# rafaelvp-db/databricks-distributed-deep-learning

Measured on AMD Instinct MI355X. Metric: ResNet-50 images/sec (whole node), higher is better.
Workload: dtype bf16

## Files before the change

### csrc/include/ddl_lds.h

```cpp
#pragma once
#include "ddl_common.h"

typedef __attribute__((address_space(3))) void lds_void;
typedef __attribute__((address_space(3))) s16x4 lds_v4;
typedef uint32_t u32x2 __attribute__((ext_vector_type(2)));
typedef uint32_t u32x4 __attribute__((ext_vector_type(4)));

#define BARRIER() __builtin_amdgcn_s_barrier()
#define LGKM0() asm volatile("s_waitcnt lgkmcnt(0)" ::: "memory")
#define VMN(n) asm volatile("s_waitcnt vmcnt(" #n ")" ::: "memory")

__device__ __forceinline__ void wait_vm(int n) {
    switch (n) {
        case 0: asm volatile("s_waitcnt vmcnt(0)" ::: "memory"); break;
        case 1: asm volatile("s_waitcnt vmcnt(1)" ::: "memory"); break;
        case 2: asm volatile("s_waitcnt vmcnt(2)" ::: "memory"); break;
        case 6: asm volatile("s_waitcnt vmcnt(6)" ::: "memory"); break;
        case 7: asm volatile("s_waitcnt vmcnt(7)" ::: "memory"); break;
        case 8: asm volatile("s_waitcnt vmcnt(8)" ::: "memory"); break;
        default: asm volatile("s_waitcnt vmcnt(0)" ::: "memory"); break;
    }
}

__device__ __forceinline__ bf16x8 ds_read16(uint32_t addr) {
    bf16x8 v;
    asm volatile("ds_read_b128 %0, %1" : "=v"(v) : "v"(addr));
    return v;
}
template <int OFF>
__device__ __forceinline__ bf16x8 ds_read16_off(uint32_t addr) {
    bf16x8 v;
    asm volatile("ds_read_b128 %0, %1 offset:%2" : "=v"(v) : "v"(addr), "i"(OFF));
    return v;
}
__device__ __forceinline__ uint2 ds_read8(uint32_t addr) {
    uint2 v;
    asm volatile("ds_read_b64 %0, %1" : "=v"(v) : "v"(addr));
    return v;
}
__device__ __forceinline__ uint32_t ds_read32(uint32_t addr) {
    uint32_t v;
    asm volatile("ds_read_b32 %0, %1" : "=v"(v) : "v"(addr));
    return v;
}
__device__ __forceinline__ void ds_write8(uint32_t addr, uint2 v) {
    asm volatile("ds_write_b64 %0, %1" ::"v"(addr), "v"(v) : "memory");
}
__device__ __forceinline__ void ds_write16(uint32_t addr, u32x4 v) {
    asm volatile("ds_write_b128 %0, %1" ::"v"(addr), "v"(v) : "memory");
}
__device__ __forceinline__ s16x4 ds_read_tr8(uint32_t addr) {
    s16x4 v;
    asm volatile("ds_read_b64_tr_b16 %0, %1" : "=v"(v) : "v"(addr));
    return v;
}
__device__ __forceinline__ bf16x8 tr_frag(uint32_t a, uint32_t b) {
    const s16x4 lo = ds_read_tr8(a), hi = ds_read_tr8(b);
    typedef short s16x8 __attribute__((ext_vector_type(8)));
    const s16x8 r = {lo[0], lo[1], lo[2], lo[3], hi[0], hi[1], hi[2], hi[3]};
    return __builtin_bit_cast(bf16x8, r);
}

__device__ __forceinline__ s16x4 lds_read_tr(lds_v4* __restrict__ p) {
    return __builtin_amdgcn_ds_read_tr16_b64_v4i16(p);
}

__device__ __forceinline__ void glds16(const void* g, char* dst) {
    __builtin_amdgcn_global_load_lds(g, (lds_void*)dst, 16, 0, 0);
}
__device__ __forceinline__ void glds16_nt(const void* g, char* dst) {
    __builtin_amdgcn_global_load_lds(g, (lds_void*)dst, 16, 0, 2);
}
__device__ __forceinline__ void glds4(const void* g, char* dst) {
    __builtin_amdgcn_global_load_lds(g, (lds_void*)dst, 4, 0, 0);
}
__device__ __forceinline__ __amdgpu_buffer_rsrc_t rsrc(const void* p, uint32_t bytes) {
    return __builtin_amdgcn_make_buffer_rsrc(const_cast<void*>(p), 0, (int)bytes, 0x00020000);
}

__device__ __forceinline__ int swz_kc(int b) { return b ^ (((b >> 9) & 1) << 5); }
__device__ __forceinline__ int swz_ko(int r) { return 2 * ((r & 3) | (((r >> 3) & 1) << 2)); }
__device__ __forceinline__ bf16x8 frag_ko(const char* img, int col_base, int lane) {
    const int g = lane >> 4, q = (lane >> 2) & 3, pq = lane & 3;
    const int chunk = (col_base + 4 * pq) >> 3;
    const int ra = 8 * g + q, rb = ra + 4;
    const s16x4 lo = lds_read_tr((lds_v4*)(img + ra * 256 + ((chunk ^ swz_ko(ra)) << 4) + (pq & 1) * 8));
    const s16x4 hi = lds_read_tr((lds_v4*)(img + rb * 256 + ((chunk ^ swz_ko(rb)) << 4) + (pq & 1) * 8));
    typedef short s16x8 __attribute__((ext_vector_type(8)));
    const s16x8 r = {lo[0], lo[1], lo[2], lo[3], hi[0], hi[1], hi[2], hi[3]};
    return __builtin_bit_cast(bf16x8, r);
}

template <int W>
constexpr int swm() { return W / 8 >= 16 ? 15 : W / 8 - 1; }

template <int NWAVES, int W, int NROWS, long LD = W>
__device__ __forceinline__ void dma_rows(const bf16_t* src, long row0, long rows_valid, char* dst, int wv, int lane) {
    constexpr int CPR = W / 8;
    constexpr int RPI = CPR >= 64 ? 1 : 64 / CPR;
    constexpr int IPR = CPR >= 64 ? CPR / 64 : 1;
    constexpr int NINST = NROWS * IPR / RPI;
    static_assert(NINST % NWAVES == 0, "instructions split evenly over the waves");
#pragma unroll
    for (int qq = 0; qq < NINST / NWAVES; ++qq) {
        const int q = qq * NWAVES + wv;
        const int r = (q / IPR) * RPI + (CPR >= 64 ? 0 : lane / CPR);
        const int cl = CPR >= 64 ? (q % IPR) * 64 + lane : lane % CPR;
        const int c = cl ^ (r & swm<W>());
        const long gr = min(row0 + r, rows_valid - 1);
        glds16_nt(src + gr * LD + c * 8, dst + q * 1024);
    }
}
```

### csrc/kernels/conv3_bwd.hip

```cpp
#include "ddl_lds.h"

#include <algorithm>

namespace {

constexpr int NW = 8, NTH = NW * 64;
constexpr int TM = 32;
constexpr int DPT = 6, SPT = 1;

struct C3Params {
    const bf16_t* dz;
    const bf16_t* x3;
    const float* mean3;
    const float* istd3;
    const float* coef3;
    const bf16_t* a2;
    const bf16_t* x2;
    const uint8_t* mask2;
    const float* mean2;
    const float* istd2;
    const bf16_t* wt;
    bf16_t* dz2;
    float* colstats;
    bf16_t* wpart;
    long M;
    int tiles, chunk;
    uint32_t dz2_bytes;
};

__device__ __forceinline__ u32x4 bn_apply8(bf16x8 dzv, bf16x8 xv, const float* A, const float* B, const float* D,
                                           bool valid) {
    const u32x4 gw = __builtin_bit_cast(u32x4, dzv), xw = __builtin_bit_cast(u32x4, xv);
    const uint32_t keep = valid ? ~0u : 0u;
    u32x4 o;
#pragma unroll
    for (int i = 0; i < 4; ++i) {
        const float g0 = lo_f(gw[i]), g1 = hi_f(gw[i]);
        const float x0 = lo_f(xw[i]), x1 = hi_f(xw[i]);
        const float o0 = bn_bwd_apply1(A[2 * i], g0, B[2 * i], x0, D[2 * i]);
        const float o1 = bn_bwd_apply1(A[2 * i + 1], g1, B[2 * i + 1], x1, D[2 * i + 1]);
        o[i] = pack2bf(o0, o1) & keep;
    }
    return o;
}

template <int CO, int CI, int NBUF>
__global__ __launch_bounds__(NTH, 1) void conv3_bwd_k(C3Params p) {
    static_assert(CO == 256 && CI == 64 && (NBUF == 2 || NBUF == 3), "shape");
    constexpr int WBYTES = CI * CO * 2, ZBYTES = TM * CO * 2, ABYTES = TM * CI * 2;
    constexpr int O_DZ = 0, O_X3 = ZBYTES, O_A2 = 2 * ZBYTES, O_X2 = O_A2 + ABYTES, O_MK = O_X2 + ABYTES;
    constexpr int BUFB = O_MK + 1024;
    constexpr int LDS = WBYTES + NBUF * BUFB;
    static_assert(LDS <= 160 * 1024, "LDS");
    __shared__ __attribute__((aligned(16))) char smem[LDS];
    const int tid = threadIdx.x, lane = tid & 63, wv = __builtin_amdgcn_readfirstlane(tid >> 6);
    const int g = lane >> 4, r16 = lane & 15;
    const uint32_t lds0 = (uint32_t)(uintptr_t)smem;
    const __amdgpu_buffer_rsrc_t crs = rsrc(p.dz2, p.dz2_bytes);
    const int t0 = blockIdx.x * p.chunk, t1 = min(p.tiles, t0 + p.chunk);

    auto prefetch = [&](int t, int buf) {
        char* base = smem + WBYTES + buf * BUFB;
        const long m0 = (long)t * TM;
#pragma unroll
        for (int qq = 0; qq < 2; ++qq) {
            const int q = qq * NW + wv, r = q * 2 + (lane >> 5), c = (lane & 31) ^ (r & 15);
            const long gr = min(m0 + r, p.M - 1);
            glds16_nt(p.dz + gr * CO + c * 8, base + O_DZ + q * 1024);
            glds16_nt(p.x3 + gr * CO + c * 8, base + O_X3 + q * 1024);
        }
        {
            const int q = wv & 3, r = q * 8 + (lane >> 3), c = (lane & 7) ^ (r & 7);
            const long gr = min(m0 + r, p.M - 1);
            glds16_nt((wv < 4 ? p.a2 : p.x2) + gr * CI + c * 8, base + (wv < 4 ? O_A2 : O_X2) + q * 1024);
        }
        {
            const long b = min(m0 * (CI / 8) + lane * 4, p.M * (CI / 8) - 4);
            const uint8_t* src = p.mask2 ? p.mask2 + b : (const uint8_t*)p.a2;
            glds4(src, base + O_MK);
        }
    };
#pragma unroll
    for (int qq = 0; qq < CI / 2 / NW; ++qq) {
        const int q = qq * NW + wv, r = q * 2 + (lane >> 5), c = (lane & 31) ^ (r & 15);
        glds16_nt(p.wt + (long)r * CO + c * 8, smem + q * 1024);
    }
#pragma unroll
    for (int u = 0; u < NBUF - 1; ++u)
        if (t0 + u < t1) prefetch(t0 + u, u);

    const int tc = tid & 31, tr = tid >> 5;
    float cA[8], cB[8], cD[8];
    bn_bwd_apply_coefs8(p.mean3, p.istd3, p.coef3, CO, tc * 8, cA, cB, cD);
    const uint32_t toff = tr * (CO * 2) + ((tc ^ tr) << 4);

    const int dj = wv & 3;
    const bool dgw = wv < 4;
    uint32_t aoff[2][CO / 32], boff[CO / 32];
#pragma unroll
    for (int kk = 0; kk < CO / 32; ++kk) {
        const int rb = 16 * dj + r16;
        boff[kk] = lds0 + rb * (CO * 2) + (((kk * 4 + g) ^ (rb & 15)) << 4);
#pragma unroll
        for (int i = 0; i < 2; ++i) {
            const int ra = 16 * i + r16;
            aoff[i][kk] = ra * (CO * 2) + (((kk * 4 + g) ^ (ra & 15)) << 4);
        }
    }
    uint32_t coff[2], moff[2];
// ... 86 lines not shown
            }
        }
        LGKM0();
        __builtin_amdgcn_sched_barrier(0);
        {
            typedef short s16x8 __attribute__((ext_vector_type(8)));
            bf16x8 fa[2], fb[4];
#pragma unroll
            for (int i = 0; i < 2; ++i) {
                const s16x8 r = {fal[i][0][0], fal[i][0][1], fal[i][0][2], fal[i][0][3],
                                 fal[i][1][0], fal[i][1][1], fal[i][1][2], fal[i][1][3]};
                fa[i] = __builtin_bit_cast(bf16x8, r);
            }
#pragma unroll
            for (int j = 0; j < 4; ++j) {
                const s16x8 r = {fbl[j][0][0], fbl[j][0][1], fbl[j][0][2], fbl[j][0][3],
                                 fbl[j][1][0], fbl[j][1][1], fbl[j][1][2], fbl[j][1][3]};
                fb[j] = __builtin_bit_cast(bf16x8, r);
            }
#pragma unroll
            for (int i = 0; i < 2; ++i)
#pragma unroll
                for (int j = 0; j < 4; ++j)
                    wacc[i][j] = __builtin_amdgcn_mfma_f32_16x16x32_bf16(fb[j], fa[i], wacc[i][j], 0, 0, 0);
        }
        if (dgw) {
#pragma unroll
            for (int i = 0; i < 2; ++i) {
                float v[4] = {acc[i][0], acc[i][1], acc[i][2], acc[i][3]};
                const float xv[4] = {lo_f(ev[i].x), hi_f(ev[i].x), lo_f(ev[i].y), hi_f(ev[i].y)};
                const uint32_t bits = mword[i] >> mshift;
#pragma unroll
                for (int e = 0; e < 4; ++e) v[e] = ((bits >> e) & 1u) ? v[e] : 0.f;
                const uint32_t lo = pack2bf(v[0], v[1]), hi = pack2bf(v[2], v[3]);
                ds_write8(img + O_X2 + coff[i], make_uint2(lo, hi));
                if (m0 + 16 * i + r16 < p.M) {
                    const float tq[4] = {lo_f(lo), hi_f(lo), lo_f(hi), hi_f(hi)};
#pragma unroll
                    for (int e = 0; e < 4; ++e) {
                        st_s[e] += tq[e];
                        st_q[e] = __builtin_fmaf(tq[e], xv[e], st_q[e]);
                    }
                }
            }
        }
        LGKM0();
        __builtin_amdgcn_s_barrier();
        {
            const int row = 4 * wv + (lane >> 4), pc = lane & 15;
            const uint2 d = ds_read8(img + O_X2 + row * (CI * 2) + (((pc >> 1) ^ (row & 7)) << 4) + (pc & 1) * 8);
            LGKM0();
            __builtin_amdgcn_sched_barrier(0);
            const long grow = m0 + row;
            const uint32_t off = grow < p.M ? (uint32_t)((grow * CI + pc * 4) * 2) : 0x80000000u;
            __builtin_amdgcn_raw_buffer_store_b64(__builtin_bit_cast(u32x2, d), crs, (int)off, 0, 0);
        }
        buf = buf + 1 == NBUF ? 0 : buf + 1;
    }
    asm volatile("s_waitcnt vmcnt(0)" ::: "memory");
    __syncthreads();

    bf16_t* wout = p.wpart + (long)blockIdx.x * CO * CI;
#pragma unroll
    for (int i = 0; i < 2; ++i)
#pragma unroll
        for (int j = 0; j < 4; ++j)
            *reinterpret_cast<uint2*>(wout + (long)(32 * wv + 16 * i + r16) * CI + 16 * j + 4 * g) =
                make_uint2(pack2bf(wacc[i][j][0], wacc[i][j][1]), pack2bf(wacc[i][j][2], wacc[i][j][3]));

    if (dgw) {
#pragma unroll
        for (int e = 0; e < 4; ++e) {
            const float a = row16_sum(st_s[e]), b = row16_sum(st_q[e]);
            if (r16 == 0) {
                const int col = 16 * dj + 4 * g + e;
                p.colstats[(long)blockIdx.x * 2 * CI + col] = a;
                p.colstats[(long)blockIdx.x * 2 * CI + CI + col] =
                    __builtin_fmaf(-p.mean2[col], a, b) * p.istd2[col];
            }
        }
    }
}

}

DDL_API int ddl_conv3_bwd_grid(long M, int grid) {
    const int tiles64 = (int)((M + 63) / 64);
    const int g = std::min(grid > 0 ? std::min(grid, 256) : 256, tiles64);
    const int chunk64 = (tiles64 + g - 1) / g;
    return (tiles64 + chunk64 - 1) / chunk64;
}

DDL_API int ddl_conv3_bwd(const void* dz, const void* x3, const float* mean3, const float* istd3, const float* coef3,
                          const void* a2, const void* x2, const uint8_t* mask2, const float* mean2, const float* istd2,
                          const void* wt, void* dz2, float* colstats, void* wpart, long wpart_elems, void* dW,
                          int dw_f32, int accumulate, long M, int Cout, int Cin, int grid, hipStream_t st) {
    if (Cout != 256 || Cin != 64 || M < 1 || M * (long)Cout * 2 >= (1l << 31)) return -1;
    if (!dz || !x3 || !mean3 || !istd3 || !coef3 || !a2 || !x2 || !mean2 || !istd2 || !wt || !dz2 || !colstats ||
        !wpart || !dW)
        return -1;
    for (const void* q : {dz, x3, a2, x2, wt, (const void*)dz2, (const void*)wpart})
        if ((uintptr_t)q & 15) return -1;
    if ((uintptr_t)dW & (dw_f32 ? 15 : 7)) return -1;
    C3Params p{};
    p.dz = (const bf16_t*)dz;
    p.x3 = (const bf16_t*)x3;
    p.mean3 = mean3;
    p.istd3 = istd3;
    p.coef3 = coef3;
    p.a2 = (const bf16_t*)a2;
    p.x2 = (const bf16_t*)x2;
    p.mask2 = mask2;
    p.mean2 = mean2;
    p.istd2 = istd2;
    p.wt = (const bf16_t*)wt;
    p.dz2 = (bf16_t*)dz2;
    p.colstats = colstats;
    p.wpart = (bf16_t*)wpart;
    p.M = M;
    p.tiles = (int)((M + TM - 1) / TM);
    const int G = ddl_conv3_bwd_grid(M, grid);
    p.chunk = 2 * (((int)((M + 63) / 64) + G - 1) / G);
    p.dz2_bytes = (uint32_t)(M * Cin * 2);
    if (wpart_elems < (long)G * Cout * Cin) return -1;
    hipLaunchKernelGGL((conv3_bwd_k<256, 64, 3>), dim3(G), dim3(NTH), 0, st, p);
    ddl_wgrad_reduce(p.wpart, G, Cout, Cin, dW, Cin, accumulate, dw_f32, st);
    const hipError_t e = hipGetLastError();
    if (e != hipSuccess) return -2 - (int)e;
    return G;
}
```

### databricks_distributed_deep_learning_amd/ops/_lib.py

```python
from __future__ import annotations

import ctypes
import os
from typing import Optional

import torch

_PKG_DIR = os.path.dirname(os.path.dirname(os.path.abspath(__file__)))
LIB_PATH = os.environ.get("DDL_NATIVE_LIB") or os.path.join(_PKG_DIR, "_native", "libddl_kernels.so")

_lib: Optional[ctypes.CDLL] = None
_load_error: Optional[str] = None
_mode = os.environ.get("DDL_NATIVE", "auto").lower()


class NativeUnavailable(RuntimeError):
    pass


def set_mode(mode: str) -> None:
    global _mode
    if mode not in ("auto", "on", "off"):
        raise ValueError(mode)
    _mode = mode
# ... 38 lines not shown
def load_error() -> Optional[str]:
    load()
    return _load_error


def use_native(*tensors: torch.Tensor) -> bool:
    if _mode == "off":
        return False
    if not all(t is None or t.is_cuda for t in tensors):
        return False
    if load() is None:
        raise NativeUnavailable(
            f"HIP kernel library unavailable on a GPU run: {_load_error}. "
            "Build it with `python csrc/build.py` or set DDL_NATIVE=off for stock PyTorch ops.")
    return True


def get() -> ctypes.CDLL:
    lib = load()
    if lib is None:
        raise NativeUnavailable(_load_error)
    return lib


def stream() -> ctypes.c_void_p:
    return ctypes.c_void_p(torch.cuda.current_stream().cuda_stream)


def ptr(t: Optional[torch.Tensor]) -> ctypes.c_void_p:
    return ctypes.c_void_p(0 if t is None else t.data_ptr())


def check(rc: int, what: str) -> None:
    if rc != 0:
        raise RuntimeError(f"native kernel {what} failed with HIP error {rc}")


P, I, L, F, U64 = ctypes.c_void_p, ctypes.c_int, ctypes.c_long, ctypes.c_float, ctypes.c_uint64
_SIGS = {
    "ddl_bn_stats_nblk": [L, I],
    "ddl_bn_bwd_nblk": [L, I],
    "ddl_bn_rows_sum": [P, I, I, P, P, P],
    "ddl_rows_sum_sink": [I, P, I, I, I, P, I, P, P],
    "ddl_bn_stats_partials": [I, P, L, I, P, P],
    "ddl_bn_bwd_partials": [I, P, P, P, P, P, L, I, I, P, P],
    "ddl_bn_bwd_finish": [I, P, P, P, P, P, P, L, L, I, I, P, P, P, P, P, P, P, I, P],
    "ddl_bn_bwd_from_partials": [I, P, I, P, L, P, P, P, P, P, L, I, P, P, P, P, P, I, P],
    "ddl_bn_partials_ws": [I, I],
    "ddl_bn_fwd_train": [I, P, L, I, P, P, P, P, F, F, P, P, P, P, P, P],
    "ddl_bn_eval_coeffs": [I, I, P, P, P, P, F, P, P, P],
    "ddl_bn_apply": [I, P, P, P, P, P, L, I, I, P, P],
    "ddl_bn_apply2": [I, P, P, P, P, P, P, P, L, I, I, P, P],
    "ddl_bn_relu_maxpool": [I, P, P, P, P, P, P, I, I, I, I, I, I, P],
    "ddl_bn_bwd_pool_nblk": [],
    "ddl_bn_bwd_pool": [I, P, P, P, P, P, P, P, I, I, I, I, I, I, P, P, P, P, P, I, P],
    "ddl_bn_bwd_coef_from_partials": [I, P, I, P, L, P, P, L, I, P, P, P, I, P],
    "ddl_bn_bwd_apply_coef": [I, P, P, P, P, P, L, I, P, P],
    "ddl_bn_fwd_from_partials": [I, P, I, L, I, P, P, P, P, F, F, P, P, P, P, P, L],
    "ddl_conv_w_dgrad": [P, P, I, I, I, I, I, I, P, P, P],
    "ddl_conv_w_dgrad_batch": [P, P, I, P],
    "ddl_gelu_bwd_colsum": [I, P, P, P, L, I, P, P, I, I, P],
    "ddl_acc_f32": [I, P, P, L, P],
    "ddl_tanh_bwd": [I, P, P, P, L, P],
    "ddl_copy2d": [I, P, L, L, L, P, L, L, L, P],
    "ddl_add_into": [I, P, P, L, P],
    "ddl_zero": [P, L, P],
    "ddl_rows_add_row": [I, P, P, P, L, L, P],
    "ddl_seq_prepend_add": [I, P, P, P, P, L, L, L, P],
    "ddl_sort_ids_ok": [L, L],
    "ddl_sort_ids": [P, L, P, P, P],
    "ddl_drain_acc": [I, P, P, L, P],
    "ddl_acc_grad": [I, P, P, L, I, I, P],
    "ddl_softmax_topk": [I, P, L, I, I, P, P, P, P],
    "ddl_gemm_conv_multi": [I, I, P, P, P, P, P, L, I, P, P],
    "ddl_conv3x3": [P, P, P, I, I, I, I, I, P, P, P, P, P, P, I, P],
    "ddl_conv3x3_wgrad": [P, P, P, I, I, I, I, I, P, L, I, I, I, P],
    "ddl_stem_wgrad": [P, P, P, I, I, I, I, I, I, I, P, L, I, I, I, P],
    "ddl_stem_fwd": [P, P, P, I, I, I, I, P, I, P],
    "ddl_s2d_input": [P, I, I, I, I, I, P, I, I, P],
    "ddl_s2d_weight": [P, I, I, I, I, P, I, I, P],
    "ddl_skinny_gemm": [P, P, P, L, I, I, P, P, P, P, P, P, I, P],
    "ddl_stream_gemm": [P, P, P, L, I, I, P, P, P, P, P, P, I, P],
    "ddl_stream_wgrad_ws": [I, I],
    "ddl_conv3_bwd_grid": [L, I],
    "ddl_conv3_bwd": [P, P, P, P, P, P, P, P, P, P, P, P, P, P, L, P, I, I, L, I, I, I, P],
    "ddl_bn_bwd": [I, P, P, P, P, P, P, L, I, I, P, P, P, P, P, P, I, P],
    "ddl_ln_supported": [I],
    "ddl_ln_fwd": [I, P, P, L, P, P, P, P, P, L, I, F, U64, F, P],
    "ddl_ln_bwd_nblk": [L],
    "ddl_ln_bwd": [I, P, P, P, L, P, P, P, P, P, P, P, L, I, I, P, U64, F, P, P, P, P],
    "ddl_gelu_fwd": [I, P, P, L, P],
    "ddl_gelu_bwd": [I, P, P, P, L, P],
    "ddl_dropout": [I, P, P, L, U64, F, P],
    "ddl_colsum_nblk": [L],
    "ddl_colsum": [I, P, L, I, P, P, I, I, P],
    "ddl_softmax_ce": [I, P, P, L, I, P, P, P, P],
    "ddl_scale_by": [I, P, P, P, L, P],
    "ddl_maxpool_fwd": [I, P, P, P, I, I, I, I, I, I, I, I, I, P],
    "ddl_maxpool_bwd": [I, P, P, P, I, I, I, I, I, I, I, I, I, P],
    "ddl_avgpool_fwd": [I, P, P, I, I, I, P],
    "ddl_avgpool_bwd": [I, P, P, I, I, I, P],
    "ddl_embedding_fwd": [I, P, P, P, L, I, P],
    "ddl_embedding_bwd": [I, P, P, P, P, L, L, I, I, P],
    "ddl_embedding_bwd_sorted": [I, P, P, P, P, P, L, I, I, P],
    "ddl_sgd_step": [I, P, P, I, P, P, P, I, P, F, F, F, I, I, P],
    "ddl_adamw_step": [I, P, P, I, P, P, P, P, I, P, F, F, F, F, F, F, F, F, F, P],
    "ddl_lamb_step": [I, P, P, I, P, P, P, P, I, P, F, F, F, F, F, F, F, F, F, P, P],
    "ddl_sumsq": [I, P, L, P, P],
    "ddl_lamb_phase1": [I, P, P, P, P, P, I, P, F, F, F, F, F, F, F, F, P, P],
    "ddl_lamb_phase2": [P, I, P, P, P, P, I, F, F, F, F, F, P, P],
}
_fns = {}


def fn(name: str):
    f = _fns.get(name)
    if f is None:
        f = getattr(get(), name)
        if name in _SIGS:
            f.argtypes = _SIGS[name]
        f.restype = ctypes.c_int
        _fns[name] = f
    return f


def call(name: str, *args) -> None:
    rc = fn(name)(*args, stream())
    if rc != 0:
        raise RuntimeError(f"native kernel {name} failed with code {rc}")


def register(sigs: dict) -> None:
    _SIGS.update(sigs)


def dcode(t: torch.Tensor) -> int:
    if t.dtype == torch.bfloat16:
        return 1
    if t.dtype == torch.float32:
        return 0
    raise TypeError(f"native kernels support fp32/bf16, got {t.dtype}")


def p(t: Optional[torch.Tensor]) -> int:
    return 0 if t is None else t.data_ptr()


def grad_sink(param) -> Optional[torch.Tensor]:
    if param is None:
        return None
    return getattr(param, "_ddl_main_grad", None)


def grad_ready(param) -> None:
    cb = getattr(param, "_ddl_grad_ready", None)
    if cb is not None:
        cb()


import contextlib as _contextlib

_WGRAD_STREAM = os.environ.get("DDL_WGRAD_STREAM", "0") != "0"
_side: dict = {}


def wgrad_stream_enabled() -> bool:
    return _WGRAD_STREAM
# ... 36 lines not shown
```

### databricks_distributed_deep_learning_amd/ops/_native_conv.py

```python
from __future__ import annotations

import ctypes
import os

import torch
import torch.nn.functional as F

from . import _lib
from ._lib import grad_ready, grad_sink
from ._native_gemm import MODE_CONV, MODE_CONVW, MODE_NN, MODE_NT, MODE_TN, gemm, plan, stats_rows_max
from ._native_norm import _BN_BWD_EPI, _BN_BWD_EPI_RES


def _desc(N, H, W, C, P, Q, stride, h_off, w_off, h_step, w_step, R, S, OH, OW, ostep=1, oa=0, ob=0):
    return [N, H, W, C, P, Q, stride, h_off, w_off, h_step, w_step, R, S, OH, OW, ostep, oa, ob]


STATS_MIN_K = int(os.environ.get("DDL_BN_STATS_MIN_K", "0"))
_DGRAD_NT = os.environ.get("DDL_DGRAD_NT", "1") != "0"


_CONV3X3 = os.environ.get("DDL_CONV3X3", "1") != "0"


# ... 328 lines not shown

_MULTI_CHOICE: dict = {}


def _pick_dgrad_path(key, serial, multi, dx):
    if not dx.is_cuda or torch.cuda.is_current_stream_capturing():
        return "serial"
    scratch = torch.empty_like(dx)
    serial(scratch)
    cands = {"serial": lambda: serial(scratch), "multi": lambda: multi(scratch, False),
             "multi_narrow": lambda: multi(scratch, True)}
    best, best_t = "serial", float("inf")
    for name, fn in cands.items():
        fn()
        e0, e1 = torch.cuda.Event(enable_timing=True), torch.cuda.Event(enable_timing=True)
        e0.record()
        for _ in range(5):
            fn()
        e1.record()
        e1.synchronize()
        t = e0.elapsed_time(e1)
        if t < best_t:
            best, best_t = name, t
    _MULTI_CHOICE[key] = best
    return best


def _direct3x3_wgrad(dy, x, dw, accumulate, grid=0):
    N, H, W_, C = x.shape
    if (tuple(dy.shape) != (N, H, W_, 64) or tuple(dw.shape) != (64, 3, 3, 64) or not dy.is_contiguous()
            or not x.is_contiguous() or not dw.is_contiguous() or dy.dtype != torch.bfloat16
            or x.dtype != torch.bfloat16 or dw.dtype not in (torch.bfloat16, torch.float32)):
        raise ValueError("direct 3x3 wgrad: operand shapes / layouts not covered")
    g = grid if grid > 0 else 256
    ws = torch.empty(g * 576 * 64, dtype=torch.float32, device=x.device)
    rc = _lib.fn("ddl_conv3x3_wgrad")(x.data_ptr(), dy.data_ptr(), dw.data_ptr(), N, H, W_, C, 64, ws.data_ptr(),
                                      ws.numel(), int(accumulate), int(dw.dtype == torch.float32), int(grid),
                                      _lib.stream())
    if rc != 0:
        raise RuntimeError(f"ddl_conv3x3_wgrad failed: {rc}")
    return dw


def _wgrad(dy, x, w_shape, stride, pad, out=None):
    N, H, W_, C = x.shape
    K, R, S, _ = w_shape
    _, P, Q, _ = dy.shape
    acc = out is not None
    dw = out if acc else torch.empty(K, R, S, C, dtype=dy.dtype, device=dy.device)
    if x.is_cuda and _direct3x3_ok(x.shape, w_shape, stride, pad) and dw.is_contiguous():
        return _direct3x3_wgrad(dy, x, dw, acc)
    M = N * P * Q
    if R == 1 and S == 1 and stride == 1 and pad == 0:
        gemm(MODE_TN, dy, K, x, C, dw, C, K, C, M, accumulate=acc)
    else:
        gemm(MODE_CONVW, dy, K, x, 0, dw, R * S * C, K, R * S * C, M, accumulate=acc,
             conv=_desc(N, H, W_, C, P, Q, stride, -pad, -pad, 1, 1, R, S, P, Q))
    return dw


def _conv3_fold_ok(x, w, stride, pad) -> bool:
    from . import bridge as B
    K, R, S, C = w.shape
    return (B.CONV3_FUSED and R == 1 and S == 1 and stride == 1 and pad == 0 and (K, C) in B.CONV3_SHAPES
            and x.is_cuda and x.dtype == torch.bfloat16 and w.dtype == torch.bfloat16 and x.is_contiguous()
            and w.is_contiguous() and x.numel() // C * K * 2 < 2 ** 31)


def _conv3_bwd_fused(parked, x, w, bnb, param, sink):
    dz, x3, mean3, istd3, coef = parked
    N, H, W_, C = x.shape
    K = w.shape[0]
    M = N * H * W_
    if (bnb is None or not _BN_BWD_EPI or tuple(bnb.x.shape) != tuple(x.shape) or not bnb.x.is_contiguous()
            or bnb.x.dtype != torch.bfloat16 or x3.numel() != M * K or dz.numel() != M * K
            or not dz.is_contiguous() or not x3.is_contiguous()
            or (bnb.mask is not None and bnb.mask.numel() * 8 < M * C)):
        return None
    if sink is not None and (not sink.is_contiguous() or sink.dtype not in (torch.bfloat16, torch.float32)):
        return None
    wt = _w_dgrad(w, [0], [0], param).view(C, K)
    dx = torch.empty(N, H, W_, C, dtype=x.dtype, device=x.device)
    dw = sink if sink is not None else torch.empty(K, 1, 1, C, dtype=x.dtype, device=x.device)
    G = _lib.fn("ddl_conv3_bwd_grid")(M, 0)
    part = torch.empty(max(stats_rows_max(M), 1024) * 2 * C + 64 * C, dtype=torch.float32, device=x.device)
    wpart = torch.empty(G * K * C, dtype=torch.bfloat16, device=x.device)
    rc = _lib.fn("ddl_conv3_bwd")(dz.data_ptr(), x3.data_ptr(), mean3.data_ptr(), istd3.data_ptr(), coef.data_ptr(),
                                  x.data_ptr(), bnb.x.data_ptr(), _lib.p(bnb.mask), bnb.mean.data_ptr(),
                                  bnb.istd.data_ptr(), wt.data_ptr(), dx.data_ptr(), part.data_ptr(),
                                  wpart.data_ptr(), wpart.numel(), dw.data_ptr(), int(dw.dtype == torch.float32),
                                  int(sink is not None), M, K, C, 0, _lib.stream())
    if rc == -1:
        return None
    if rc < 0:
        raise RuntimeError(f"ddl_conv3_bwd failed: {rc}")
    bnb.set(dx, part, rc)
    return dx, (None if sink is not None else dw)


def _conv3_materialise(parked, dy):
    from .bridge import Conv3Fold
    dz, x3, mean3, istd3, coef = parked
    C = x3.shape[-1]
    dx3 = torch.empty_like(x3)
    _lib.call("ddl_bn_bwd_apply_coef", 1, dz.data_ptr(), x3.data_ptr(), mean3.data_ptr(), istd3.data_ptr(),
              coef.data_ptr(), x3.numel() // C, C, dx3.data_ptr())
    if Conv3Fold.is_parked(parked, dy):
        return dx3
    return (dy - dz.view_as(dy)) + dx3.view_as(dy)


class _Conv(torch.autograd.Function):
    @staticmethod
    def forward(ctx, x, w, stride, pad, bridge=None, stats=None, grad_to=None):
        ctx.w_param = w
        ctx.bridge = bridge
        ctx.grad_to = grad_to
        ctx.c3 = None
        ctx.bnb = getattr(x, "_ddl_bnb", None) if grad_to is None else None
        x = x.contiguous()
        w = w.contiguous()
        ctx.stride, ctx.pad = stride, pad
        ctx.save_for_backward(x, w)
        y = _fwd(x, w, stride, pad, stats=stats)
        if _conv3_fold_ok(x, w, stride, pad) and y.is_contiguous():
            from .bridge import Conv3Fold
            ctx.c3 = y._ddl_c3 = Conv3Fold()
        return y

    @staticmethod
    def backward(ctx, dy):
        x, w = ctx.saved_tensors
        dy = dy.contiguous()
        dx = dw = None
        parked = ctx.c3.take() if ctx.c3 is not None else None
        if parked is not None:
            from .bridge import Conv3Fold
            if (Conv3Fold.is_parked(parked, dy) and ctx.needs_input_grad[0] and ctx.needs_input_grad[1]
                    and ctx.bridge is None and ctx.grad_to is None):
                sink = grad_sink(ctx.w_param)
                if sink is not None and sink.shape != w.shape:
                    sink = None
                out = _conv3_bwd_fused(parked, x, w, ctx.bnb, ctx.w_param, sink)
                if out is not None:
                    ctx.bnb = None
                    if sink is not None:
                        grad_ready(ctx.w_param)
                    return out[0], out[1], None, None, None, None, None
            dy = _conv3_materialise(parked, dy)
        del parked
        fork = _lib.fork_event() if ctx.needs_input_grad[1] else None
        if ctx.needs_input_grad[0]:
            res = ctx.bridge.take() if ctx.bridge is not None else None
            if res is not None:
                res = res.contiguous().view(x.shape)
            dx = _dgrad(dy, w, x.shape, ctx.stride, ctx.pad, residual=res, bnb=ctx.bnb, param=ctx.w_param)
            ctx.bnb = None
            if ctx.grad_to is not None and ctx.grad_to.offer(dx):
                dx = None
        if ctx.needs_input_grad[1]:
            sink = grad_sink(ctx.w_param)
            if sink is not None and sink.shape == w.shape:
                with _lib.side_stream(dy, x, after=fork):
                    _wgrad(dy, x, w.shape, ctx.stride, ctx.pad, out=sink)
                grad_ready(ctx.w_param)
            else:
                dw = _wgrad(dy, x, w.shape, ctx.stride, ctx.pad)
# ... 206 lines not shown
```

### databricks_distributed_deep_learning_amd/ops/bridge.py

```python
from __future__ import annotations

import os
from typing import Optional

import torch

CONV3_FUSED = os.environ.get("DDL_CONV3_BWD_FUSED", "1") != "0"
CONV3_SHAPES = ((256, 64),)


class GradBridge:
    __slots__ = ("grad", "closed")

    def __init__(self):
        self.grad: Optional[torch.Tensor] = None
        self.closed = False

    def put(self, g: torch.Tensor) -> None:
        if self.grad is not None:
            raise RuntimeError("GradBridge: gradient already pending (bridge reused within one backward?)")
        self.grad = g

    def offer(self, g: torch.Tensor) -> bool:
        if self.closed:
            return False
        self.put(g)
        return True

    def take(self) -> Optional[torch.Tensor]:
        g, self.grad = self.grad, None
        self.closed = True
        return g


class _BridgeJoin(torch.autograd.Function):

    @staticmethod
    def forward(ctx, x, bridge):
        ctx.bridge = bridge
        return x.view_as(x)

    @staticmethod
    def backward(ctx, g):
        r = ctx.bridge.take()
        return (g if r is None else g + r.view_as(g)), None


def join(x: torch.Tensor, bridge: Optional[GradBridge]) -> torch.Tensor:
    return x if bridge is None else _BridgeJoin.apply(x, bridge)


class BNStats:
    __slots__ = ("ptr", "numel", "part", "nblk")

    def __init__(self):
        self.ptr = None
        self.numel = 0
        self.part = None
        self.nblk = 0

    def set(self, y: torch.Tensor, part: torch.Tensor, nblk: int) -> None:
        self.ptr, self.numel, self.part, self.nblk = y.data_ptr(), y.numel(), part, nblk

    def take_for(self, x: torch.Tensor):
        if self.part is None or self.ptr != x.data_ptr() or self.numel != x.numel():
            return None
        part, nblk = self.part, self.nblk
        self.part = None
        return part, nblk


class BNBackward:
    __slots__ = ("x", "mask", "mean", "istd", "dz", "part", "nrows")

    def __init__(self, x: torch.Tensor, mask: Optional[torch.Tensor], mean: torch.Tensor, istd: torch.Tensor):
        self.x, self.mask, self.mean, self.istd = x, mask, mean, istd
        self.dz = None
        self.part = None
        self.nrows = 0

    def set(self, dz: torch.Tensor, part: torch.Tensor, nrows: int) -> None:
        self.dz, self.part, self.nrows = dz, part, nrows

    def take_for(self, g: torch.Tensor):
        dz, part, nrows = self.dz, self.part, self.nrows
        self.dz = self.part = None
        if dz is None or dz.data_ptr() != g.data_ptr() or dz.numel() != g.numel():
            return None
        return part, nrows


# ... 21 lines not shown
```

Baseline: 13020.

## Extend fused conv3 backward kernel to stage-2 bottleneck shape via channel slabs

Adds a new fused backward kernel for the 512->128 bottleneck conv3 (BN backward apply, dgrad GEMM, ReLU mask, BN2 stats and weight-gradient partials) that splits the 128 input channels into two 64-wide slabs handled by paired blocks with a double-buffered LDS ring. The Python side enables the fused path for this shape by default, so stage-2 layers avoid separate BN-backward, dgrad and wgrad launches and their intermediate memory traffic. The cost is that each slab block re-reads and re-normalises the full dz/x3 rows, which duplicates that work across the two slabs, plus higher LDS use and lower occupancy.

```diff
diff --git a/csrc/include/ddl_lds.h b/csrc/include/ddl_lds.h
--- a/csrc/include/ddl_lds.h
+++ b/csrc/include/ddl_lds.h
@@ -52,6 +52,12 @@
 __device__ __forceinline__ s16x4 ds_read_tr8(uint32_t addr) {
     s16x4 v;
     asm volatile("ds_read_b64_tr_b16 %0, %1" : "=v"(v) : "v"(addr));
+    return v;
+}
+template <int OFF>
+__device__ __forceinline__ s16x4 ds_read_tr8_off(uint32_t addr) {
+    s16x4 v;
+    asm volatile("ds_read_b64_tr_b16 %0, %1 offset:%2" : "=v"(v) : "v"(addr), "i"(OFF));
     return v;
 }
 __device__ __forceinline__ bf16x8 tr_frag(uint32_t a, uint32_t b) {
diff --git a/csrc/kernels/conv3_bwd.hip b/csrc/kernels/conv3_bwd.hip
--- a/csrc/kernels/conv3_bwd.hip
+++ b/csrc/kernels/conv3_bwd.hip
@@ -1,6 +1,7 @@
 #include "ddl_lds.h"
 
 #include <algorithm>
+#include <type_traits>
 
 namespace {
 
@@ -25,6 +26,7 @@
     bf16_t* wpart;
     long M;
     int tiles, chunk;
+    int nchunks;
     uint32_t dz2_bytes;
 };
 
@@ -277,9 +279,254 @@
     }
 }
 
-}
-
-DDL_API int ddl_conv3_bwd_grid(long M, int grid) {
+template <int NBUF>
+__global__ __launch_bounds__(NTH, 1) void conv3_bwd_slab_k(C3Params p) {
+    constexpr int CO = 512, CI = 128, SL = 64;
+    static_assert(NBUF == 2, "ring");
+    constexpr int ZBYTES = TM * CO * 2, ABYTES = TM * SL * 2;
+    constexpr int O_DZ = 0, O_X3 = ZBYTES, O_A2 = 2 * ZBYTES, O_X2 = O_A2 + ABYTES, O_MK = O_X2 + ABYTES;
+    constexpr int BUFB = O_MK + 1024;
+    constexpr int LDS = NBUF * BUFB;
+    static_assert(LDS <= 160 * 1024 && BUFB % 256 == 0 && O_A2 % 256 == 0, "LDS");
+    __shared__ __attribute__((aligned(256))) char smem[LDS];
+    const int tid = threadIdx.x, lane = tid & 63, wv = __builtin_amdgcn_readfirstlane(tid >> 6);
+    const int g = lane >> 4, r16 = lane & 15;
+    const int slab = (int)((blockIdx.x >> 3) & 1);
+    const int chunk = (int)((blockIdx.x & 7) + 8 * (blockIdx.x >> 4));
+    if (chunk >= p.nchunks) return;
+    const int n0 = slab * SL;
+    const uint32_t lds0 = (uint32_t)(uintptr_t)smem;
+    const __amdgpu_buffer_rsrc_t crs = rsrc(p.dz2, p.dz2_bytes);
+    const int t0 = chunk * p.chunk, t1 = min(p.tiles, t0 + p.chunk);
+
+    auto prefetch = [&](int t, int buf) {
+        char* base = smem + buf * BUFB;
+        const long m0 = (long)t * TM;
+#pragma unroll
+        for (int qq = 0; qq < 4; ++qq) {
+            const int r = qq * NW + wv, c = lane ^ (r & 15);
+            const long gr = min(m0 + r, p.M - 1);
+            glds16(p.dz + gr * CO + c * 8, base + O_DZ + r * 1024);
+            glds16(p.x3 + gr * CO + c * 8, base + O_X3 + r * 1024);
+        }
+        {
+            const int q = wv & 3, r = q * 8 + (lane >> 3), c = (lane & 7) ^ (r & 7);
+            const long gr = min(m0 + r, p.M - 1);
+            glds16_nt((wv < 4 ? p.a2 : p.x2) + gr * CI + n0 + c * 8, base + (wv < 4 ? O_A2 : O_X2) + q * 1024);
+        }
+        {
+            const long gr = min(m0 + (lane >> 1), p.M - 1);
+            const uint8_t* src = p.mask2 ? p.mask2 + gr * (CI / 8) + n0 / 8 + 4 * (lane & 1) : (const uint8_t*)p.a2;
+            glds4(src, base + O_MK);
+        }
+    };
+
+    const int dj = wv & 3;
+    const bool dgw = wv < 4;
+    bf16x8 breg[CO / 32];
+    if (dgw) {
+#pragma unroll
+        for (int kk = 0; kk < CO / 32; ++kk)
+            breg[kk] = *reinterpret_cast<const bf16x8*>(p.wt + (long)(n0 + 16 * dj + r16) * CO + 32 * kk + 8 * g);
+    }
+    if (t0 < t1) prefetch(t0, 0);
+
+    const int tc = lane;
+    float cA[8], cB[8], cD[8];
+    bn_bwd_apply_coefs8(p.mean3, p.istd3, p.coef3, CO, tc * 8, cA, cB, cD);
+    const uint32_t toff0 = wv * (CO * 2) + ((tc ^ wv) << 4);
+    const uint32_t toff1 = (wv + 8) * (CO * 2) + ((tc ^ (wv + 8)) << 4);
+
+    const uint32_t ab = r16 * (CO * 2) + ((g ^ r16) << 4);
+    uint32_t coff[2], moff[2];
+#pragma unroll
+    for (int i = 0; i < 2; ++i) {
+        const int drow = 16 * i + r16;
+        coff[i] = drow * (SL * 2) + (((2 * dj + (g >> 1)) ^ (drow & 7)) << 4) + (g & 1) * 8;
+        moff[i] = drow * (SL / 8) + (dj >> 1) * 4;
+    }
+    const int mshift = (dj & 1) * 16 + 4 * g;
+    float st_s[4] = {0.f, 0.f, 0.f, 0.f}, st_q[4] = {0.f, 0.f, 0.f, 0.f};
+
+    const int q4 = (lane >> 2) & 3, pq = lane & 3;
+    const int wr = 8 * g + q4;
+    const uint32_t wa = wr * (CO * 2) + (((8 * wv + (pq >> 1)) ^ (wr & 15)) << 4) + (pq & 1) * 8;
+    const uint32_t wb = wr * (SL * 2) + (((pq >> 1) ^ (wr & 7)) << 4) + (pq & 1) * 8;
+    f32x4 wacc[4][4];
+#pragma unroll
+    for (int i = 0; i < 4; ++i)
+#pragma unroll
+        for (int j = 0; j < 4; ++j) wacc[i][j] = (f32x4){0.f, 0.f, 0.f, 0.f};
+
+    __builtin_amdgcn_s_waitcnt(0xF70);
+    for (int t = t0; t < t1; ++t) {
+        const int buf = (t - t0) & 1;
+        wait_vm(t > t0 ? SPT : 0);
+        __builtin_amdgcn_s_barrier();
+        if (t + 1 < t1) prefetch(t + 1, buf ^ 1);
+        const uint32_t img = lds0 + buf * BUFB;
+        const long m0 = (long)t * TM;
+
+        {
+            const uint32_t a0 = img + O_DZ + toff0, a1 = img + O_DZ + toff1;
+            const bf16x8 z0 = ds_read16(a0), z1 = ds_read16(a1);
+            const bf16x8 z2 = ds_read16_off<16 * CO * 2>(a0), z3 = ds_read16_off<16 * CO * 2>(a1);
+            const bf16x8 x0 = ds_read16_off<ZBYTES>(a0), x1 = ds_read16_off<ZBYTES>(a1);
+            const bf16x8 x2 = ds_read16_off<ZBYTES + 16 * CO * 2>(a0), x3 = ds_read16_off<ZBYTES + 16 * CO * 2>(a1);
+            LGKM0();
+            __builtin_amdgcn_sched_barrier(0);
+            ds_write16(a0, bn_apply8(z0, x0, cA, cB, cD, m0 + wv < p.M));
+            ds_write16(a1, bn_apply8(z1, x1, cA, cB, cD, m0 + wv + 8 < p.M));
+            ds_write16(a0 + 16 * CO * 2, bn_apply8(z2, x2, cA, cB, cD, m0 + wv + 16 < p.M));
+            ds_write16(a1 + 16 * CO * 2, bn_apply8(z3, x3, cA, cB, cD, m0 + wv + 24 < p.M));
+            LGKM0();
+            __builtin_amdgcn_s_barrier();
+        }
+
+        f32x4 acc[2] = {{0.f, 0.f, 0.f, 0.f}, {0.f, 0.f, 0.f, 0.f}};
+        if (dgw) {
+            const uint32_t aimg = img + ab;
+            auto ksteps = [&](auto KH) __attribute__((always_inline)) {
+                constexpr int kh = decltype(KH)::value;
+                bf16x8 af[2][4];
+#pragma unroll
+                for (int kl = 0; kl < 4; ++kl) {
+                    af[0][kl] = ds_read16_off<O_DZ + 256 * kh>(aimg ^ (kl << 6));
+                    af[1][kl] = ds_read16_off<O_DZ + 256 * kh + 16 * CO * 2>(aimg ^ (kl << 6));
+                }
+                LGKM0();
+                __builtin_amdgcn_sched_barrier(0);
+#pragma unroll
+                for (int kl = 0; kl < 4; ++kl) {
+                    acc[0] = __builtin_amdgcn_mfma_f32_16x16x32_bf16(breg[4 * kh + kl], af[0][kl], acc[0], 0, 0, 0);
+                    acc[1] = __builtin_amdgcn_mfma_f32_16x16x32_bf16(breg[4 * kh + kl], af[1][kl], acc[1], 0, 0, 0);
+                }
+                __builtin_amdgcn_sched_barrier(0);
+            };
+            ksteps(std::integral_constant<int, 0>{});
+            ksteps(std::integral_constant<int, 1>{});
+            ksteps(std::integral_constant<int, 2>{});
+            ksteps(std::integral_constant<int, 3>{});
+        }
+        s16x4 fal[4][2], fbl[4][2];
+        {
+            const uint32_t waimg = img + wa, wbimg = img + O_A2 + wb;
+#pragma unroll
+            for (int i = 0; i < 4; ++i) {
+                fal[i][0] = ds_read_tr8_off<O_DZ>(waimg ^ (i << 5));
+                fal[i][1] = ds_read_tr8_off<O_DZ + 4 * CO * 2>(waimg ^ (i << 5) ^ 64);
+            }
+#pragma unroll
+            for (int j = 0; j < 4; ++j) {
+                fbl[j][0] = ds_read_tr8_off<0>(wbimg ^ (j << 5));
+                fbl[j][1] = ds_read_tr8_off<4 * SL * 2>(wbimg ^ (j << 5) ^ 64);
+            }
+        }
+        uint32_t mword[2] = {~0u, ~0u};
+        uint2 ev[2] = {make_uint2(0u, 0u), make_uint2(0u, 0u)};
+        if (dgw) {
+#pragma unroll
+            for (int i = 0; i < 2; ++i) {
+                if (p.mask2) mword[i] = ds_read32(img + O_MK + moff[i]);
+                ev[i] = ds_read8(img + O_X2 + coff[i]);
+            }
+        }
+        LGKM0();
+        __builtin_amdgcn_sched_barrier(0);
+        {
+            typedef short s16x8 __attribute__((ext_vector_type(8)));
+            bf16x8 fa[4], fb[4];
+#pragma unroll
+            for (int i = 0; i < 4; ++i) {
+                const s16x8 r = {fal[i][0][0], fal[i][0][1], fal[i][0][2], fal[i][0][3],
+                                 fal[i][1][0], fal[i][1][1], fal[i][1][2], fal[i][1][3]};
+                fa[i] = __builtin_bit_cast(bf16x8, r);
+            }
+#pragma unroll
+            for (int j = 0; j < 4; ++j) {
+                const s16x8 r = {fbl[j][0][0], fbl[j][0][1], fbl[j][0][2], fbl[j][0][3],
+                                 fbl[j][1][0], fbl[j][1][1], fbl[j][1][2], fbl[j][1][3]};
+                fb[j] = __builtin_bit_cast(bf16x8, r);
+            }
+#pragma unroll
+            for (int i = 0; i < 4; ++i)
+#pragma unroll
+                for (int j = 0; j < 4; ++j)
+                    wacc[i][j] = __builtin_amdgcn_mfma_f32_16x16x32_bf16(fb[j], fa[i], wacc[i][j], 0, 0, 0);
+        }
+        if (dgw) {
+#pragma unroll
+            for (int i = 0; i < 2; ++i) {
+                float v[4] = {acc[i][0], acc[i][1], acc[i][2], acc[i][3]};
+                const float xv[4] = {lo_f(ev[i].x), hi_f(ev[i].x), lo_f(ev[i].y), hi_f(ev[i].y)};
+                const uint32_t bits = mword[i] >> mshift;
+#pragma unroll
+                for (int e = 0; e < 4; ++e) v[e] = ((bits >> e) & 1u) ? v[e] : 0.f;
+                const uint32_t lo = pack2bf(v[0], v[1]), hi = pack2bf(v[2], v[3]);
+                ds_write8(img + O_X2 + coff[i], make_uint2(lo, hi));
+                if (m0 + 16 * i + r16 < p.M) {
+                    const float tq[4] = {lo_f(lo), hi_f(lo), lo_f(hi), hi_f(hi)};
+#pragma unroll
+                    for (int e = 0; e < 4; ++e) {
+                        st_s[e] += tq[e];
+                        st_q[e] += tq[e] * xv[e];
+                    }
+                }
+            }
+        }
+        LGKM0();
+        __builtin_amdgcn_s_barrier();
+        {
+            const int row = 4 * wv + (lane >> 4), pc = lane & 15;
+            const uint2 d = ds_read8(img + O_X2 + row * (SL * 2) + (((pc >> 1) ^ (row & 7)) << 4) + (pc & 1) * 8);
+            LGKM0();
+            __builtin_amdgcn_sched_barrier(0);
+            const long grow = m0 + row;
+            const uint32_t off = grow < p.M ? (uint32_t)((grow * CI + n0 + pc * 4) * 2) : 0x80000000u;
+            __builtin_amdgcn_raw_buffer_store_b64(__builtin_bit_cast(u32x2, d), crs, (int)off, 0, 0);
+        }
+    }
+    asm volatile("s_waitcnt vmcnt(0)" ::: "memory");
+    __syncthreads();
+
+    bf16_t* wout = p.wpart + (long)chunk * CO * CI + n0;
+#pragma unroll
+    for (int i = 0; i < 4; ++i)
+#pragma unroll
+        for (int j = 0; j < 4; ++j)
+            *reinterpret_cast<uint2*>(wout + (long)(64 * wv + 16 * i + r16) * CI + 16 * j + 4 * g) =
+                make_uint2(pack2bf(wacc[i][j][0], wacc[i][j][1]), pack2bf(wacc[i][j][2], wacc[i][j][3]));
+
+    if (dgw) {
+#pragma unroll
+        for (int e = 0; e < 4; ++e) {
+            float a = row16_sum(st_s[e]), b = row16_sum(st_q[e]);
+            const int col = n0 + 16 * dj + 4 * g + e;
+            b = (b - p.mean2[col] * a) * p.istd2[col];
+            if (r16 == 0) {
+                p.colstats[(long)chunk * 2 * CI + col] = a;
+                p.colstats[(long)chunk * 2 * CI + CI + col] = b;
+            }
+        }
+    }
+}
+
+int slab_chunks(long M, int grid, int* chunk) {
+    const int tiles = (int)((M + TM - 1) / TM);
+    const int c = std::min(grid > 0 ? std::min(grid, 256) : 256, tiles);
+    *chunk = (tiles + c - 1) / c;
+    return (tiles + *chunk - 1) / *chunk;
+}
+
+}
+
+DDL_API int ddl_conv3_bwd_grid(long M, int Cout, int Cin, int grid) {
+    if (M < 1) return 0;
+    if (Cout == 512 && Cin == 128) {
+        int chunk;
+        return slab_chunks(M, grid, &chunk);
+    }
+    if (Cout != 256 || Cin != 64) return 0;
     const int tiles64 = (int)((M + 63) / 64);
     const int g = std::min(grid > 0 ? std::min(grid, 256) : 256, tiles64);
     const int chunk64 = (tiles64 + g - 1) / g;
@@ -290,7 +537,8 @@
                           const void* a2, const void* x2, const uint8_t* mask2, const float* mean2, const float* istd2,
                           const void* wt, void* dz2, float* colstats, void* wpart, long wpart_elems, void* dW,
                           int dw_f32, int accumulate, long M, int Cout, int Cin, int grid, hipStream_t st) {
-    if (Cout != 256 || Cin != 64 || M < 1 || M * (long)Cout * 2 >= (1l << 31)) return -1;
+    const bool st1 = Cout == 256 && Cin == 64, st2 = Cout == 512 && Cin == 128;
+    if ((!st1 && !st2) || M < 1 || M * (long)Cout * 2 >= (1l << 31)) return -1;
     if (!dz || !x3 || !mean3 || !istd3 || !coef3 || !a2 || !x2 || !mean2 || !istd2 || !wt || !dz2 || !colstats ||
         !wpart || !dW)
         return -1;
@@ -314,11 +562,16 @@
     p.wpart = (bf16_t*)wpart;
     p.M = M;
     p.tiles = (int)((M + TM - 1) / TM);
-    const int G = ddl_conv3_bwd_grid(M, grid);
-    p.chunk = 2 * (((int)((M + 63) / 64) + G - 1) / G);
+    const int G = ddl_conv3_bwd_grid(M, Cout, Cin, grid);
     p.dz2_bytes = (uint32_t)(M * Cin * 2);
     if (wpart_elems < (long)G * Cout * Cin) return -1;
-    hipLaunchKernelGGL((conv3_bwd_k<256, 64, 3>), dim3(G), dim3(NTH), 0, st, p);
+    if (st2) {
+        p.nchunks = slab_chunks(M, grid, &p.chunk);
+        hipLaunchKernelGGL((conv3_bwd_slab_k<2>), dim3(2 * ((G + 7) / 8 * 8)), dim3(NTH), 0, st, p);
+    } else {
+        p.chunk = 2 * (((int)((M + 63) / 64) + G - 1) / G);
+        hipLaunchKernelGGL((conv3_bwd_k<256, 64, 3>), dim3(G), dim3(NTH), 0, st, p);
+    }
     ddl_wgrad_reduce(p.wpart, G, Cout, Cin, dW, Cin, accumulate, dw_f32, st);
     const hipError_t e = hipGetLastError();
     if (e != hipSuccess) return -2 - (int)e;
diff --git a/databricks_distributed_deep_learning_amd/ops/_lib.py b/databricks_distributed_deep_learning_amd/ops/_lib.py
--- a/databricks_distributed_deep_learning_amd/ops/_lib.py
+++ b/databricks_distributed_deep_learning_amd/ops/_lib.py
@@ -144,7 +144,7 @@
     "ddl_skinny_gemm": [P, P, P, L, I, I, P, P, P, P, P, P, I, P],
     "ddl_stream_gemm": [P, P, P, L, I, I, P, P, P, P, P, P, I, P],
     "ddl_stream_wgrad_ws": [I, I],
-    "ddl_conv3_bwd_grid": [L, I],
+    "ddl_conv3_bwd_grid": [L, I, I, I],
     "ddl_conv3_bwd": [P, P, P, P, P, P, P, P, P, P, P, P, P, P, L, P, I, I, L, I, I, I, P],
     "ddl_bn_bwd": [I, P, P, P, P, P, P, L, I, I, P, P, P, P, P, P, I, P],
     "ddl_ln_supported": [I],
diff --git a/databricks_distributed_deep_learning_amd/ops/_native_conv.py b/databricks_distributed_deep_learning_amd/ops/_native_conv.py
--- a/databricks_distributed_deep_learning_amd/ops/_native_conv.py
+++ b/databricks_distributed_deep_learning_amd/ops/_native_conv.py
@@ -434,7 +434,7 @@
     wt = _w_dgrad(w, [0], [0], param).view(C, K)
     dx = torch.empty(N, H, W_, C, dtype=x.dtype, device=x.device)
     dw = sink if sink is not None else torch.empty(K, 1, 1, C, dtype=x.dtype, device=x.device)
-    G = _lib.fn("ddl_conv3_bwd_grid")(M, 0)
+    G = _lib.fn("ddl_conv3_bwd_grid")(M, K, C, 0)
     part = torch.empty(max(stats_rows_max(M), 1024) * 2 * C + 64 * C, dtype=torch.float32, device=x.device)
     wpart = torch.empty(G * K * C, dtype=torch.bfloat16, device=x.device)
     rc = _lib.fn("ddl_conv3_bwd")(dz.data_ptr(), x3.data_ptr(), mean3.data_ptr(), istd3.data_ptr(), coef.data_ptr(),
diff --git a/databricks_distributed_deep_learning_amd/ops/bridge.py b/databricks_distributed_deep_learning_amd/ops/bridge.py
--- a/databricks_distributed_deep_learning_amd/ops/bridge.py
+++ b/databricks_distributed_deep_learning_amd/ops/bridge.py
@@ -6,7 +6,7 @@
 import torch
 
 CONV3_FUSED = os.environ.get("DDL_CONV3_BWD_FUSED", "1") != "0"
-CONV3_SHAPES = ((256, 64),)
+CONV3_SHAPES = ((256, 64),) if os.environ.get("DDL_CONV3_BWD_FUSED") == "stage1" else ((256, 64), (512, 128))
 
 
 class GradBridge:
```

New measurement: 13080 (median of 6 runs). No clear change (+0.5%).
